# microscopic-image-analysis/geosss

Hardware: AMD Instinct MI355X
Metric: mcmc_chain_steps_per_sec (higher is better)
Workload: dtype f64; 1 GPU; vmfmix_readme: shrinkage slice sampler, 1000000 chains/GPU x 1000 transitions per launch, thin=100; target=vmfmix_readme, d=3, chains_per_gpu=1000000, thin=100, mode=fast, kernel=screened_kernel<3, ScreenVmf<3, 3>>, kept_rows_layout=components, slice_steps=128, library_matches_tree=True, stream=philox-v3 (chain,step)-keyed; S2: tangent = one angle; 32-bit tries

## Files before the change

### geosss_amd/_lib.py

```python
import ctypes as C
import os

_HERE = os.path.dirname(os.path.abspath(__file__))
LIB_PATH = os.environ.get("GSSS_HIP_LIB") or os.path.join(_HERE, "libgsss_hip.so")

VMF_MIXTURE, BINGHAM, CURVE_VMF, CPD, MIXTURE, USER = 1, 2, 3, 4, 5, 6
SHRINK, REJECT, RWMH, HMC, INDEP, MIX = 0, 1, 2, 3, 4, 5
MODE_EXACT, MODE_FAST = 0, 1
VARIANT_FAST_DOUBLE = 100
VARIANT_FAST_VERIFY = 101
CHAIN_MAX_TRIES, CHAIN_NONFINITE, CHAIN_REPLAY_EXHAUSTED, CHAIN_COUNTER_SATURATED = 1, 2, 4, 8
ABI_VERSION = 10
STATS_NO_SECOND_MOMENT = 1
MOMENTS_DIAG = 1


class GsssError(RuntimeError):
    pass


class TargetDesc(C.Structure):
    _fields_ = [("kind", C.c_int32), ("d", C.c_int32), ("k", C.c_int32), ("reserved", C.c_int32),
                ("mu", C.c_void_p), ("logc", C.c_void_p), ("A", C.c_void_p), ("knots", C.c_void_p),
                ("kappa", C.c_double),
                ("source", C.c_void_p), ("source_w", C.c_void_p), ("target", C.c_void_p), ("target_w", C.c_void_p),
                ("n_target", C.c_int32), ("target_dim", C.c_int32), ("k_nn", C.c_int32), ("outlier", C.c_int32),
                ("sigma", C.c_double), ("beta", C.c_double), ("omega", C.c_double), ("log_volume", C.c_double)]


class RunArgs(C.Structure):
    _fields_ = [("state_dev", C.c_void_p), ("samples_dev", C.c_void_p), ("n_reject_dev", C.c_void_p),
                ("n_tries_dev", C.c_void_p), ("err_dev", C.c_void_p), ("replay_dev", C.c_void_p),
                ("replay_stride", C.c_int64), ("n_chains", C.c_int64), ("n_steps", C.c_int64), ("thin", C.c_int64),
                ("seed", C.c_uint64), ("chain_offset", C.c_uint64), ("step_offset", C.c_uint64),
                ("sampler", C.c_int32), ("mode", C.c_int32), ("max_tries", C.c_int32), ("variant", C.c_int32),
                ("rng_state_dev", C.c_void_p), ("samples_chain_rows", C.c_int64), ("placement", C.c_int32),
                ("stats_lags", C.c_int32), ("stats_dev", C.c_void_p), ("stats_dirs_dev", C.c_void_p),
                ("stats_modes", C.c_int32), ("n_leapfrog", C.c_int32), ("stepsize_dev", C.c_void_p),
                ("n_accept_dev", C.c_void_p), ("momenta_dev", C.c_void_p), ("adapt_steps", C.c_int64),
                ("mixing_probability", C.c_double), ("adapt_left_dev", C.c_void_p), ("n_rwmh_dev", C.c_void_p),
                ("momenta_samples_dev", C.c_void_p), ("stepsize_trace_dev", C.c_void_p), ("stats_flags", C.c_int32),
                ("reserved0", C.c_int32)]


SIGNATURES = {
    "gsss_abi_version": (C.c_int, []),
    "gsss_last_error": (C.c_char_p, []),
    "gsss_source_digest": (C.c_char_p, []),
    "gsss_device_count": (C.c_int, []),
    "gsss_target_create": (C.c_int, [C.POINTER(TargetDesc), C.c_int, C.POINTER(C.c_void_p)]),
    "gsss_target_create_mixture": (C.c_int, [C.POINTER(TargetDesc), C.c_int32, C.c_void_p, C.c_int, C.POINTER(C.c_void_p)]),
    "gsss_target_create_batch": (C.c_int, [C.POINTER(TargetDesc), C.c_int32, C.c_int64, C.c_int, C.POINTER(C.c_void_p)]),
    "gsss_exact_layout": (C.c_int, [C.c_int32]),
    "gsss_target_create_user": (C.c_int, [C.c_void_p, C.c_int32, C.c_void_p, C.c_int64, C.c_int, C.POINTER(C.c_void_p)]),
    "gsss_target_destroy": (C.c_int, [C.c_void_p]),
    "gsss_target_dim": (C.c_int, [C.c_void_p]),
    "gsss_logprob": (C.c_int, [C.c_void_p, C.c_void_p, C.c_int64, C.c_void_p, C.c_void_p]),
    "gsss_gradient": (C.c_int, [C.c_void_p, C.c_void_p, C.c_int64, C.c_void_p, C.c_void_p]),
    "gsss_run": (C.c_int, [C.c_void_p, C.POINTER(RunArgs), C.c_void_p]),
    "gsss_stats_rows": (C.c_int64, [C.c_int32, C.c_int32, C.c_int32, C.c_int32]),
    "gsss_moments_rows": (C.c_int64, [C.c_int32, C.c_int32]),
    "gsss_target_moments": (C.c_int, [C.c_void_p, C.c_int64, C.c_int64, C.c_int32, C.c_int64, C.c_int64, C.c_int32, C.c_void_p,
                                      C.c_void_p, C.c_int, C.c_void_p]),
    "gsss_batch_logprob": (C.c_int, [C.c_void_p, C.c_void_p, C.c_int64, C.c_void_p, C.c_void_p]),
    "gsss_batch_gradient": (C.c_int, [C.c_void_p, C.c_void_p, C.c_int64, C.c_void_p, C.c_void_p]),
    "gsss_batch_logprob_draws": (C.c_int, [C.c_void_p, C.c_void_p, C.c_int64, C.c_int64, C.c_int64, C.c_void_p, C.c_void_p]),
    "gsss_scalar_moments": (C.c_int, [C.c_void_p, C.c_int64, C.c_int64, C.c_int64, C.c_void_p, C.c_void_p, C.c_int, C.c_void_p]),
    "gsss_last_launch": (C.c_int, [C.POINTER(C.c_int64), C.POINTER(C.c_int32), C.POINTER(C.c_double)]),
    "gsss_batch_plan": (C.c_int, [C.c_int32, C.c_int32, C.c_int32, C.c_int32, C.c_int64, C.c_int64, C.POINTER(C.c_int32),
                                  C.POINTER(C.c_int32), C.POINTER(C.c_int64), C.POINTER(C.c_double)]),
    "gsss_mode_supported": (C.c_int, [C.c_void_p, C.c_int32]),
    "gsss_variant_name": (C.c_char_p, [C.c_void_p, C.c_int32, C.c_int32]),
    "gsss_kernel_name": (C.c_char_p, [C.c_void_p, C.c_int32, C.c_int32, C.c_int32]),
    "gsss_sample_sphere": (C.c_int, [C.c_uint64, C.c_uint64, C.c_int64, C.c_int32, C.c_void_p, C.c_int, C.c_void_p]),
    "gsss_tangent_s2": (C.c_int, [C.c_void_p, C.c_void_p, C.c_int64, C.c_int32, C.c_void_p, C.c_int, C.c_void_p]),
    "gsss_screen_constants": (C.c_int, [C.POINTER(C.c_double), C.c_int32]),
    "gsss_f32_error_sweep": (C.c_int, [C.c_int32, C.POINTER(C.c_double), C.POINTER(C.c_uint64), C.c_int, C.c_void_p]),
    "gsss_rows_to_components": (C.c_int, [C.c_void_p, C.c_void_p, C.c_int64, C.c_int32, C.c_int, C.c_void_p]),
    "gsss_components_to_rows": (C.c_int, [C.c_void_p, C.c_void_p, C.c_int64, C.c_int32, C.c_int, C.c_void_p]),
    "gsss_samples_to_chains": (C.c_int, [C.c_void_p, C.c_void_p, C.c_int64, C.c_int64, C.c_int32, C.c_int, C.c_void_p]),
    "gsss_malloc": (C.c_int, [C.POINTER(C.c_void_p), C.c_size_t, C.c_int]),
    "gsss_free": (C.c_int, [C.c_void_p, C.c_int]),
    "gsss_memcpy_h2d": (C.c_int, [C.c_void_p, C.c_void_p, C.c_size_t, C.c_int, C.c_void_p]),
    "gsss_memcpy_d2h": (C.c_int, [C.c_void_p, C.c_void_p, C.c_size_t, C.c_int, C.c_void_p]),
    "gsss_malloc_host": (C.c_int, [C.POINTER(C.c_void_p), C.c_size_t, C.c_int]),
    "gsss_free_host": (C.c_int, [C.c_void_p]),
    "gsss_host_register": (C.c_int, [C.c_void_p, C.c_size_t, C.c_int]),
    "gsss_host_unregister": (C.c_int, [C.c_void_p]),
    "gsss_memcpy_d2h_async": (C.c_int, [C.c_void_p, C.c_void_p, C.c_size_t, C.c_int, C.c_void_p]),
    "gsss_memset": (C.c_int, [C.c_void_p, C.c_int, C.c_size_t, C.c_int, C.c_void_p]),
    "gsss_stream_synchronize": (C.c_int, [C.c_int, C.c_void_p]),
}

_lib = None


def load():
    global _lib
    if _lib is not None:
        return _lib
    if not os.path.exists(LIB_PATH):
        raise GsssError(f"{LIB_PATH} is missing: build it with `python -m geosss_amd.build` "
                        "(there is no CPU fallback for the sampler)")
    lib = C.CDLL(LIB_PATH)
    for name, (res, args) in SIGNATURES.items():
        fn = getattr(lib, name)
        fn.restype = res
        fn.argtypes = args
    if lib.gsss_abi_version() != ABI_VERSION:
        raise GsssError(f"libgsss_hip.so has ABI {lib.gsss_abi_version()}, binding expects {ABI_VERSION}")
    _lib = lib
    return lib


def check(code):
    if code != 0:
        msg = load().gsss_last_error().decode("utf-8", "replace")
        if code in (-1, -2):
            raise ValueError(f"gsss: {msg} (code {code})")
        raise GsssError(f"gsss: {msg} (code {code})")


def require_device():
    lib = load()
    n = lib.gsss_device_count()
    if n <= 0:
        raise GsssError("no HIP device visible: the geodesic slice sampler runs on MI355X only "
                        "(no CPU fallback is provided)")
    return n
```

### geosss_amd/csrc/gsss_capi.hip

```cpp
#include <cmath>
#include <cstdarg>
#include <cstdio>
#include <cstring>
#include <mutex>
#include <new>
#include <string>
#include <vector>

#include "gsss_batch.h"
#include "gsss_batch_logprob.h"
#include "gsss_fast.h"
#include "gsss_launch.h"
#include "gsss_mh.h"
#include "gsss_moments.h"
#include "gsss_user_target.h"

namespace gsss {

static thread_local char g_err[512] = "";

static thread_local LaunchInfo g_last_launch = {0, 0, 0.0};
LaunchInfo &last_launch() { return g_last_launch; }

int64_t resident_workgroups(const void *kern, size_t lds_bytes, int *per_cu_out)
{
    struct Entry {
        const void *kern;
        size_t lds;
        int dev, per_cu, cus;
    };
    static std::mutex mu;
    static std::vector<Entry> cache;
    int dev = 0;
    if (hipGetDevice(&dev) != hipSuccess) {
        (void)hipGetLastError();
        return 0;
    }
    const char *env = getenv("GSSS_RESIDENT_PER_CU");
    const int forced = env ? atoi(env) : 0;
    int per_cu = 0, cus = 0;
    {
        std::lock_guard<std::mutex> lock(mu);
        for (const Entry &e : cache)
            if (e.kern == kern && e.lds == lds_bytes && e.dev == dev) {
                per_cu = e.per_cu;
                cus = e.cus;
                break;
            }
    }
    if (per_cu < 1) {
        if (hipOccupancyMaxActiveBlocksPerMultiprocessor(&per_cu, kern, kBlock, lds_bytes) != hipSuccess || per_cu < 1 ||
            hipDeviceGetAttribute(&cus, hipDeviceAttributeMultiprocessorCount, dev) != hipSuccess || cus < 1) {
            (void)hipGetLastError();
            return 0;
        }
        std::lock_guard<std::mutex> lock(mu);
        cache.push_back(Entry{kern, lds_bytes, dev, per_cu, cus});
    }
    if (forced > 0) per_cu = forced;
    if (per_cu_out) *per_cu_out = per_cu;
    return (int64_t)per_cu * cus;
}

void slice_fallback_note(const char *why)
{
    if (getenv("GSSS_DEBUG_OCCUPANCY")) fprintf(stderr, "gsss: %s\n", why);
}

void set_error(const char *fmt, ...)
{
    va_list ap;
    va_start(ap, fmt);
    vsnprintf(g_err, sizeof(g_err), fmt, ap);
    va_end(ap);
}

static const VecInfo kVecs[] = {
#define GSSS_VEC_ROW(ID, V, NAME) {ID, V::L, V::N, V::DPAD, V::kExactDim, NAME},
    GSSS_VEC_LIST(GSSS_VEC_ROW)
#undef GSSS_VEC_ROW
};

const VecInfo *vec_table(int *count)
{
    *count = (int)(sizeof(kVecs) / sizeof(kVecs[0]));
    return kVecs;
}

int select_vec(int d, int variant)
{
    int n;
    const VecInfo *v = vec_table(&n);
    if (variant != 0) {
        for (int i = 0; i < n; ++i)
            if (v[i].id == variant) {
                if (v[i].exact_dim ? v[i].dpad == d : d <= v[i].dpad) return variant;
                set_error("kernel variant %s does not cover d=%d", v[i].name, d);
                return GSSS_E_UNSUPPORTED;
            }
        set_error("unknown kernel variant %d", variant);
        return GSSS_E_INVALID;
    }
    for (int i = 0; i < n; ++i)
        if (v[i].exact_dim && v[i].dpad == d) return v[i].id;
    for (int i = 0; i < n; ++i)
        if (!v[i].exact_dim && d <= v[i].dpad) return v[i].id;
    set_error("no kernel variant covers d=%d (max %d)", d, v[n - 1].dpad);
    return GSSS_E_UNSUPPORTED;
}

static int select_vec_for(const gsss::TargetBlock &tb, int variant)
{
    const int vec = select_vec(tb.d, variant);
    if (vec < 0 || variant != 0) return vec;
    int n;
    const VecInfo *v = vec_table(&n);
    size_t dpad = 0;
    for (int i = 0; i < n; ++i)
        if (v[i].id == vec) dpad = (size_t)v[i].dpad;
    if (dpad >= 256) return vec;
    size_t rows = 0;
    if (tb.kind == GSSS_MIXTURE) {
        int L = 1;
        for (int i = 0; i < n; ++i)
            if (v[i].id == vec) L = v[i].L;
        const MixInfo mi = mix_info(tb);
        const size_t need = (size_t)mi.n * 8 + (L > 1 ? (dpad + 1) * (size_t)(kBlock / L) : 0) + kMixDrawsReserve +
                            (size_t)mi.rows * dpad + (size_t)mi.extra;
        if (need * sizeof(double) <= kMaxLdsBytes) return vec;
        for (int i = 0; i < n; ++i)
            if (!v[i].exact_dim && v[i].dpad >= 256 && tb.d <= v[i].dpad) return v[i].id;
        return vec;
    }
    switch (tb.kind) {
    case GSSS_VMF_MIXTURE: rows = (size_t)tb.k * dpad + (size_t)tb.k; break;
    case GSSS_BINGHAM: rows = (size_t)(tb.d + 1) * dpad; break;
    case GSSS_CURVE_VMF: rows = (size_t)tb.k * dpad + 4 * (size_t)(tb.k - 1); break;
    default: return vec;
    }
    if (rows * sizeof(double) <= gsss::kRowsLdsBytes) return vec;
    for (int i = 0; i < n; ++i)
        if (!v[i].exact_dim && v[i].dpad >= 256 && tb.d <= v[i].dpad) return v[i].id;
    return vec;
}
// ... 981 lines not shown
        const int served = fast_select(fast_ask(t, rb.screen, rb.spread != 0, numpy, replay, rb.stats != nullptr), pick);
        if (numpy && (served != GSSS_OK || !pick.lane)) {
            set_error("in fast mode the numpy stream is served by the lane-per-chain kernels only (gsss_variant_name: "
                      "\"fast-lane\"); use GSSS_MODE_EXACT");
            return GSSS_E_UNSUPPORTED;
        }
        if (a->n_steps > 0x7FFFFFFFll || a->thin > 0x7FFFFFFFll || a->n_chains > 0x7FFFFFFFll - 1024 ||
            a->replay_stride > 0x7FFFFFFFll) {
            set_error("fast mode takes at most 2^31-1 steps / chains per call");
            return GSSS_E_INVALID;
        }
        if (served != GSSS_OK) return fast_refused(t);
        return fast_launch(pick, t->tb, rb, t->batch, replay, st);
    }
    if (mh) {
        if (a->rng_state_dev && (a->sampler == GSSS_RWMH || a->sampler == GSSS_MIX) && t->tb.d < 3) {
            set_error("numpy's gamma(1) is an exponential ziggurat, not restated: RWMH on numpy's stream needs d >= 3");
            return GSSS_E_UNSUPPORTED;
        }
        MhBlock mb;
        mb.stepsize = a->stepsize_dev;
        mb.n_accept = a->n_accept_dev;
        mb.momenta = a->sampler == GSSS_HMC ? a->momenta_dev : nullptr;
        mb.adapt_steps = a->adapt_steps;
        mb.n_leapfrog = a->n_leapfrog;
        mb.kind = a->sampler;
        mb.mix_alpha = a->mixing_probability;
        mb.adapt_left = a->adapt_left_dev;
        mb.n_rwmh = a->n_rwmh_dev;
        mb.momenta_samples = a->sampler == GSSS_HMC ? a->momenta_samples_dev : nullptr;
        mb.stepsize_trace = a->sampler == GSSS_HMC ? nullptr : a->stepsize_trace_dev;
        if (t->tb.kind == GSSS_CPD) return launch_cpd_mh(t->cpd_variant, draws, a->sampler, t->tb, rb, mb, st);
        if (t->tb.kind == GSSS_USER) {
            if (a->sampler == GSSS_HMC && !t->user->has_gradient) {
                set_error("spherical HMC needs the target's gradient: this user target defines no gsss_user_gradient");
                return GSSS_E_UNSUPPORTED;
            }
            return t->user->mh(draws, a->sampler, t->tb, rb, mb, st);
        }
        switch (t->tb.kind) {
        case GSSS_VMF_MIXTURE: return launch_mh<VmfMixture>(vec, draws, a->sampler, t->tb, rb, mb, st);
        case GSSS_BINGHAM: return launch_mh<Bingham>(vec, draws, a->sampler, t->tb, rb, mb, st);
        case GSSS_CURVE_VMF: return launch_mh<CurveVmf>(vec, draws, a->sampler, t->tb, rb, mb, st);
        case GSSS_MIXTURE: return launch_mh<Mixture>(vec, draws, a->sampler, t->tb, rb, mb, st);
        }
        set_error("corrupt target");
        return GSSS_E_INVALID;
    }
    if (t->tb.kind == GSSS_CPD) {
        if (a->stats_dev) {
            set_error("running statistics are not built for registration targets");
            return GSSS_E_UNSUPPORTED;
        }
        return launch_cpd_run(t->cpd_variant, draws, t->tb, rb, st);
    }
    switch (t->tb.kind) {
    case GSSS_VMF_MIXTURE: return launch_run<VmfMixture>(vec, draws, t->tb, rb, st);
    case GSSS_BINGHAM: return launch_run<Bingham>(vec, draws, t->tb, rb, st);
    case GSSS_CURVE_VMF: return launch_run<CurveVmf>(vec, draws, t->tb, rb, st);
    case GSSS_MIXTURE: return launch_run<Mixture>(vec, draws, t->tb, rb, st);
    case GSSS_USER: return t->user->run(draws, t->tb, rb, st);
    }
    set_error("corrupt target");
    return GSSS_E_INVALID;
}

int gsss_batch_plan(int32_t kind, int32_t d, int32_t k, int32_t has_b, int64_t n_targets, int64_t m, int32_t *chains_per_workgroup,
                    int32_t *targets_per_workgroup, int64_t *grid, double *lane_use)
{
    (void)has_b;
    BatchPlan bp;
    if (batch_plan(kind, d, k, n_targets, m, bp) != GSSS_OK) {
        set_error("no fast-mode batch kernel for kind %d, d=%d, k=%d with %lld targets of %lld chains (vMF mixtures: d = 3 .. 10 with "
                  "K <= 16, d = 11 .. 16 with K <= 10; Bingham: d = 3 .. 16)", kind, d, k, (long long)n_targets, (long long)m);
        return GSSS_E_UNSUPPORTED;
    }
    if (chains_per_workgroup) *chains_per_workgroup = bp.per_block;
    if (targets_per_workgroup) *targets_per_workgroup = bp.targets;
    if (grid) *grid = bp.grid;
    if (lane_use) *lane_use = bp.lane_use;
    return GSSS_OK;
}

int gsss_last_launch(int64_t *grid_out, int32_t *slice_steps_out, double *sliced_fraction_out)
{
    if (grid_out) *grid_out = last_launch().grid;
    if (slice_steps_out) *slice_steps_out = last_launch().slice_steps;
    if (sliced_fraction_out) *sliced_fraction_out = last_launch().sliced_fraction;
    return GSSS_OK;
}

int64_t gsss_stats_rows(int32_t d, int32_t n_modes, int32_t n_lags, int32_t flags)
{
    if (d < 2 || n_modes < 0 || n_lags < 0 || (flags & ~GSSS_STATS_NO_SECOND_MOMENT)) return GSSS_E_INVALID;
    const int64_t second = (flags & GSSS_STATS_NO_SECOND_MOMENT) ? 0 : (int64_t)d * (d + 1) / 2;
    return 1 + 2 * (int64_t)d + second + 2 + n_modes + 2 + 3 * (int64_t)n_lags;
}

int64_t gsss_moments_rows(int32_t d, int32_t flags)
{
    if (d < 2 || (flags & ~GSSS_MOMENTS_DIAG)) return GSSS_E_INVALID;
    const bool diag = (flags & GSSS_MOMENTS_DIAG) != 0;
    if (!diag && d > kMomentsMaxFullDim) return GSSS_E_UNSUPPORTED;
    return 1 + moments_sums(d, diag);
}

int gsss_target_moments(const double *samples_dev, int64_t n_rows, int64_t n_chains, int32_t d, int64_t samples_chain_rows,
                        int64_t chains_per_target, int32_t flags, double *acc_dev, double *chain_sum_dev, int device, void *stream)
{
    if (d < 2 || (flags & ~GSSS_MOMENTS_DIAG)) {
        set_error("gsss_target_moments: need d >= 2 and known flags (d = %d, flags = %d)", d, flags);
        return GSSS_E_INVALID;
    }
    if (chains_per_target < 1 || n_chains < 0 || n_chains % chains_per_target != 0) {
        set_error("gsss_target_moments: n_chains (%lld) must be a multiple of chains_per_target (%lld) >= 1", (long long)n_chains,
                  (long long)chains_per_target);
        return GSSS_E_INVALID;
    }
    if (n_rows < 0 || samples_chain_rows < 0 || (samples_chain_rows > 0 && samples_chain_rows < n_rows)) {
        set_error("gsss_target_moments: need n_rows >= 0 and samples_chain_rows 0 or >= n_rows (%lld rows, %lld per chain)",
                  (long long)n_rows, (long long)samples_chain_rows);
        return GSSS_E_INVALID;
    }
    if (!samples_dev || !acc_dev) {
        set_error("gsss_target_moments: %s is null", samples_dev ? "acc_dev" : "samples_dev");
        return GSSS_E_INVALID;
    }
    const bool diag = (flags & GSSS_MOMENTS_DIAG) != 0;
    if (!diag && d > kMomentsMaxFullDim) {
        set_error("gsss_target_moments: the full second-moment triangle is kept for d <= %d (d = %d): pass GSSS_MOMENTS_DIAG",
                  kMomentsMaxFullDim, d);
        return GSSS_E_UNSUPPORTED;
    }
    if (n_rows == 0 || n_chains == 0) return GSSS_OK;
    DeviceGuard guard(device);
    if (!guard.ok) return GSSS_E_HIP;
    return launch_target_moments(samples_dev, n_rows, n_chains, d, samples_chain_rows, chains_per_target, diag, acc_dev, chain_sum_dev,
                                 static_cast<hipStream_t>(stream));
}

int gsss_scalar_moments(const double *values_dev, int64_t n_rows, int64_t n_chains, int64_t chains_per_target, double *acc_dev,
                        double *chain_sum_dev, int device, void *stream)
{
    if (chains_per_target < 1 || n_chains < 0 || n_chains % chains_per_target != 0) {
        set_error("gsss_scalar_moments: n_chains (%lld) must be a multiple of chains_per_target (%lld) >= 1", (long long)n_chains,
                  (long long)chains_per_target);
        return GSSS_E_INVALID;
    }
    if (n_rows < 0) {
        set_error("gsss_scalar_moments: need n_rows >= 0 (%lld)", (long long)n_rows);
        return GSSS_E_INVALID;
    }
    if (n_rows == 0 || n_chains == 0) return GSSS_OK;
    if (!values_dev || !acc_dev) {
        set_error("gsss_scalar_moments: %s is null", values_dev ? "acc_dev" : "values_dev");
        return GSSS_E_INVALID;
    }
    DeviceGuard guard(device);
    if (!guard.ok) return GSSS_E_HIP;
    return launch_target_moments(values_dev, n_rows, n_chains, 1, 0, chains_per_target, true, acc_dev, chain_sum_dev,
                                 static_cast<hipStream_t>(stream));
}

int gsss_mode_supported(const gsss_target *t, int32_t mode)
{
    if (!t) return 0;
// ... 194 lines not shown
```

### geosss_amd/csrc/gsss_device.h

```cpp
#pragma once
#include <hip/hip_runtime.h>
#include <stdint.h>
#include <stdlib.h>

#include "../../include/gsss.h"
#include "gsss_math.h"

namespace gsss {

constexpr int kBlock = 256;
constexpr double kTwoPi = 6.283185307179586;

struct TargetBlock {
    const double *blob;
    int32_t kind, d, k, dpad;
    double kappa;
    double scale;
};

struct RunBlock {
    double *state;
    double *samples;
    int64_t *n_reject;
    int64_t *n_tries;
    int32_t *err;
    const double *replay;
    uint64_t *rng_state;
    int64_t replay_stride;
    int64_t n_chains, n_steps, thin;
    uint64_t seed, chain_offset, step_offset;
    int32_t sampler, max_tries;
    int64_t keep_rows;
    int32_t spread;
    int32_t one_per_lane;
    int32_t stage_rows;
    int32_t screen;
    double *stats;
    const double *stats_dirs;
    int32_t stats_lags, stats_modes;
    int32_t stats_flags;
    int32_t stats_onchip;
    uint32_t *sched;
    int32_t slice_steps;
    int32_t sched_first;
};

struct BatchBlock {
    int64_t stride;
    int32_t m;
    int32_t chunks;
};
struct BatchShared {
    int64_t stride;
    int32_t m;
    int32_t per_block;
};
template <class... BB>
inline constexpr bool kIsBatchShared = false;
template <>
inline constexpr bool kIsBatchShared<BatchShared> = true;
template <class T>
__device__ __forceinline__ const T &first_of(const T &x)
{
    return x;
}

struct SliceSched {
    __device__ static __forceinline__ uint32_t chunks(const RunBlock &a, int per_block) { return (uint32_t)((a.n_chains + per_block - 1) / per_block); }
    __device__ static __forceinline__ uint32_t *progress(const RunBlock &a) { return a.sched + 2; }
    __device__ static __forceinline__ int32_t *dead(const RunBlock &a, int per_block)
    {
        return reinterpret_cast<int32_t *>(a.sched + 2 + chunks(a, per_block));
    }
    __device__ static __forceinline__ bool take(const RunBlock &a, int per_block, uint32_t *word, uint32_t &chunk, int32_t &s_begin,
                                                int32_t &len, bool &timed_out)
    {
        if (threadIdx.x == 0) *word = __hip_atomic_fetch_add(a.sched, 1u, __ATOMIC_RELAXED, __HIP_MEMORY_SCOPE_AGENT);
        __syncthreads();
        const uint32_t t = (uint32_t)__builtin_amdgcn_readfirstlane((int)*word);
        const uint32_t n_chunks = chunks(a, per_block) - (uint32_t)a.sched_first;
        const int32_t ss = a.slice_steps, n_steps = (int32_t)a.n_steps;
        const int32_t first_len = ss - (int32_t)(a.step_offset % (uint64_t)ss);
        const int32_t rest = n_steps - first_len;
        const uint32_t n_items = n_chunks * (uint32_t)(1 + (rest > 0 ? (rest + ss - 1) / ss : 0));
        if (t >= n_items) return false;
        const uint32_t slice = t / n_chunks;
        chunk = (uint32_t)a.sched_first + (t - slice * n_chunks);
        if (threadIdx.x == 0) {
            word[1] = chunk;
            word[2] = slice;
        }
        s_begin = slice == 0 ? 0 : first_len + (int32_t)(slice - 1) * ss;
        int32_t s_end = first_len + (int32_t)slice * ss;
        s_end = s_end < n_steps ? s_end : n_steps;
        len = s_end - s_begin;
        timed_out = false;
        if (slice > 0) {
            __syncthreads();
            if (threadIdx.x == 0) {
                uint32_t ok = 1;
                uint64_t spins = 0;
                const uint64_t limit = (uint64_t)(slice + 1u < 8u ? slice + 1u : 8u) << 22;
                while (__hip_atomic_load(progress(a) + chunk, __ATOMIC_RELAXED, __HIP_MEMORY_SCOPE_AGENT) < slice) {
                    __builtin_amdgcn_s_sleep(32);
                    if (++spins > limit) {
                        ok = 0;
                        break;
                    }
                }
                __builtin_amdgcn_fence(__ATOMIC_ACQUIRE, "agent");
                asm volatile("s_waitcnt vmcnt(0)" ::: "memory");
                *word = ok;
            }
            __syncthreads();
            timed_out = __builtin_amdgcn_readfirstlane((int)*word) == 0;
        }
        return true;
    }
    template <bool kWrittenThrough = false>
    __device__ static __forceinline__ void publish(const RunBlock &a, const uint32_t *word)
    {
        asm volatile("s_waitcnt vmcnt(0)" ::: "memory");
        __syncthreads();
        if (threadIdx.x == 0) {
            if (!kWrittenThrough) {
                __builtin_amdgcn_fence(__ATOMIC_RELEASE, "agent");
                asm volatile("s_waitcnt vmcnt(0)" ::: "memory");
            }
            __hip_atomic_store(progress(a) + word[1], word[2] + 1u, __ATOMIC_RELAXED, __HIP_MEMORY_SCOPE_AGENT);
        }
    }
    template <class T>
    __device__ static __forceinline__ void hand_over(T *p, T v)
    {
        __hip_atomic_store(p, v, __ATOMIC_RELAXED, __HIP_MEMORY_SCOPE_AGENT);
    }
};

constexpr size_t slice_sched_bytes(int64_t n_chunks, int64_t n_chains) { return 4 * (size_t)(2 + n_chunks + n_chains); }

void set_error(const char *fmt, ...);
constexpr size_t kDefaultLdsBytes = 48 * 1024;
constexpr size_t kMaxLdsBytes = 160 * 1024;
constexpr int64_t ceil_div(int64_t a, int64_t b) { return (a + b - 1) / b; }

template <class Kern>
int allow_lds(const char *family, Kern kern, size_t lds)
{
    if (lds <= kDefaultLdsBytes) return GSSS_OK;
    const hipError_t e = hipFuncSetAttribute(reinterpret_cast<const void *>(kern), hipFuncAttributeMaxDynamicSharedMemorySize, (int)lds);
    if (e == hipSuccess) return GSSS_OK;
    set_error("%s kernel: raising its dynamic LDS to %zu B failed: %s", family, lds, hipGetErrorString(e));
    return GSSS_E_HIP;
}

template <class Kern, class... Args>
int launch_kernel(const char *family, Kern kern, int64_t grid, size_t lds, hipStream_t st, void *ws, const Args &...args)
{
    hipLaunchKernelGGL(kern, dim3((unsigned)grid), dim3(kBlock), lds, st, args...);
    const hipError_t e = hipGetLastError();
    if (ws) (void)hipFreeAsync(ws, st);
    if (e == hipSuccess) return GSSS_OK;
    set_error("%s kernel launch failed: %s", family, hipGetErrorString(e));
    return GSSS_E_HIP;
}

struct SlicePlan {
    uint32_t *ws = nullptr;
    int64_t grid = 0;
    int32_t slice_steps = 0;
};
constexpr int kMaxSlices = 64;
inline int slice_length(int64_t n_steps)
{
    const char *env = getenv("GSSS_SLICE_STEPS");
    const int env_val = env ? atoi(env) : 128;
    if (env_val <= 0) return 0;
    int64_t steps = ((int64_t)env_val + 63) / 64 * 64;
    const int64_t floor_steps = ((n_steps + kMaxSlices - 1) / kMaxSlices + 63) / 64 * 64;
    if (steps < floor_steps) steps = floor_steps;
    return steps < 0x40000000ll ? (int)steps : 0;
}
int64_t resident_workgroups(const void *kern, size_t lds_bytes, int *per_cu_out = nullptr);
void slice_fallback_note(const char *why);
struct LaunchInfo {
    int64_t grid;
    int32_t slice_steps;
    double sliced_fraction;
};
LaunchInfo &last_launch();
template <class Kern>
inline SlicePlan plan_slices(Kern kern, size_t lds_bytes, const RunBlock &rb, int64_t n_chunks, bool allowed, hipStream_t st)
{
    SlicePlan p;
    p.grid = n_chunks;
    last_launch() = LaunchInfo{n_chunks, 0, 0.0};
    if (!allowed) return p;
    const int env_steps = slice_length(rb.n_steps);
    if (env_steps <= 0 || rb.n_steps < 2 * (int64_t)env_steps) return p;
    const int64_t resident = resident_workgroups(reinterpret_cast<const void *>(kern), lds_bytes);
    if (resident < 1) return p;
    const int64_t n_slices = 2 + rb.n_steps / env_steps;
    if (n_chunks <= resident || n_chunks * n_slices >= 0x7FFFFFFFll || rb.n_chains >= 0x7FFFFFFFll) return p;
    const size_t bytes = slice_sched_bytes(n_chunks, rb.n_chains);
    void *ws = nullptr;
    if (hipMallocAsync(&ws, bytes, st) != hipSuccess || ws == nullptr) {
        (void)hipGetLastError();
        slice_fallback_note("hipMallocAsync of the slice workspace failed: launching unsliced");
        return p;
    }
    if (hipMemsetAsync(ws, 0, bytes, st) != hipSuccess) {
        (void)hipGetLastError();
        (void)hipFreeAsync(ws, st);
        return p;
    }
    const int64_t first_len = env_steps - (int64_t)(rb.step_offset % (uint64_t)env_steps), rest = rb.n_steps - first_len;
    p.ws = static_cast<uint32_t *>(ws);
    p.grid = n_chunks * (1 + (rest > 0 ? (rest + env_steps - 1) / env_steps : 0));
    p.slice_steps = env_steps;
    last_launch() = LaunchInfo{p.grid, p.slice_steps, 1.0};
    return p;
}

template <class Kern>
inline SlicePlan plan_partial_round(Kern kern, size_t lds_bytes, const RunBlock &rb, int64_t n_chunks, bool allowed, hipStream_t st,
                                    int32_t &first_out)
{
    SlicePlan p;
    p.grid = n_chunks;
    first_out = 0;
    last_launch() = LaunchInfo{n_chunks, 0, 0.0};
    if (!allowed) return p;
    const int env_steps = slice_length(rb.n_steps);
    if (env_steps <= 0 || rb.n_steps < 2 * (int64_t)env_steps) return p;
    const int64_t resident = resident_workgroups(reinterpret_cast<const void *>(kern), lds_bytes);
    if (resident < 1) return p;
    const int64_t rem = n_chunks % resident, first = n_chunks - rem;
    if (n_chunks <= resident || rem == 0 || 4 * rem > 3 * resident || rb.n_chains >= 0x7FFFFFFFll) return p;
    const int64_t first_len = env_steps - (int64_t)(rb.step_offset % (uint64_t)env_steps), rest = rb.n_steps - first_len;
    const int64_t n_slices = 1 + (rest > 0 ? (rest + env_steps - 1) / env_steps : 0);
    if (rem * n_slices >= 0x7FFFFFFFll) return p;
    const size_t bytes = slice_sched_bytes(n_chunks, rb.n_chains);
    void *ws = nullptr;
    if (hipMallocAsync(&ws, bytes, st) != hipSuccess || ws == nullptr) {
        (void)hipGetLastError();
        slice_fallback_note("hipMallocAsync of the slice workspace failed: launching unsliced");
        return p;
    }
    if (hipMemsetAsync(ws, 0, bytes, st) != hipSuccess) {
        (void)hipGetLastError();
        (void)hipFreeAsync(ws, st);
        return p;
    }
    p.ws = static_cast<uint32_t *>(ws);
    p.grid = first + rem * n_slices;
    p.slice_steps = env_steps;
    first_out = (int32_t)first;
    last_launch() = LaunchInfo{p.grid, p.slice_steps, (double)rem / (double)n_chunks};
    return p;
}

__device__ __forceinline__ size_t sample_index(const RunBlock &a, int64_t row, int j, int d, int64_t c)
{
    return a.keep_rows > 0 ? ((size_t)c * a.keep_rows + row) * d + j : ((size_t)row * d + j) * a.n_chains + c;
}

template <int D>
__device__ __forceinline__ void stats_update(const RunBlock &a, int64_t c, const double (&x)[D])
{
    const size_t n = (size_t)a.n_chains;
    double *s = a.stats + c;
    const int K = a.stats_modes, L = a.stats_lags;
    const bool second = !(a.stats_flags & GSSS_STATS_NO_SECOND_MOMENT);
    const int T = second ? D * (D + 1) / 2 : 0;
    const int r_prev = 1, r_sum = 1 + D, r_xx = 1 + 2 * D, r_dist = r_xx + T, r_hop = r_dist + 1, r_mode = r_hop + 1;
    const int r_p = r_mode + K, r_lag = r_p + 2, r_ring = r_lag + L, r_head = r_ring + L;
    const double *w = a.stats_dirs, *h = a.stats_dirs + D, *modes = a.stats_dirs + 2 * D;
    const int64_t cnt = (int64_t)s[0];
    double p = 0.0, xh = 0.0;
#pragma unroll
    for (int j = 0; j < D; ++j) {
        p = fma(x[j], w[j], p);
        xh = fma(x[j], h[j], xh);
    }
    if (cnt > 0) {
        double dot = 0.0, ph = 0.0;
#pragma unroll
        for (int j = 0; j < D; ++j) {
            const double pj = s[(size_t)(r_prev + j) * n];
            dot = fma(pj, x[j], dot);
            ph = fma(pj, h[j], ph);
        }
        s[(size_t)r_dist * n] += acos(fmin(fmax(dot, -1.0), 1.0));
        const int sa = (xh > 0.0) - (xh < 0.0), sb = (ph > 0.0) - (ph < 0.0);
        if (sa != sb) s[(size_t)r_hop * n] += 1.0;
    }
    int t = 0;
#pragma unroll
    for (int i = 0; i < D; ++i) {
        s[(size_t)(r_prev + i) * n] = x[i];
        s[(size_t)(r_sum + i) * n] += x[i];
        if (second) {
#pragma unroll
            for (int j = i; j < D; ++j) s[(size_t)(r_xx + t++) * n] += x[i] * x[j];
        }
    }
    if (K > 0) {
        int best = 0;
        double bv = -INFINITY;
        for (int k = 0; k < K; ++k) {
            double v = 0.0;
#pragma unroll
            for (int j = 0; j < D; ++j) v = fma(x[j], modes[k * D + j], v);
            if (v > bv) {
                bv = v;
// ... 1434 lines not shown
```

### geosss_amd/csrc/gsss_screen.h

```cpp
#pragma once
#include <type_traits>

#include "gsss_fast.h"
#include "gsss_screen_consts.h"

namespace gsss {

enum : int32_t { kFinalAccept = 3, kFinalDecide = 4, kFinalInHi = 2 };
__device__ __forceinline__ bool is_final(int32_t st) { return st >= kFinalAccept; }
__device__ __forceinline__ bool is_decide(int32_t st) { return st == kFinalDecide || st == kFinalDecide + kFinalInHi; }

__device__ __forceinline__ void sincos_rev32(double theta, float &s, float &c)
{
    const float t = (float)(theta * 0.15915494309189535);
    s = __builtin_amdgcn_sinf(t);
    c = __builtin_amdgcn_cosf(t);
}

__device__ __forceinline__ float log2_32(double v)
{
    int e;
    const double m = frexp(v, &e);
    return (float)e + __builtin_amdgcn_logf((float)m);
}
// ... 565 lines not shown
        if (__hip_atomic_fetch_add(&gsss_svc_ticket, 1u, __ATOMIC_ACQ_REL, __HIP_MEMORY_SCOPE_AGENT) == waves - 1) {
            unsigned long long s[8];
            for (int i = 0; i < 8; ++i) s[i] = __hip_atomic_exchange(&gsss_svc_count[i], 0ull, __ATOMIC_RELAXED, __HIP_MEMORY_SCOPE_AGENT);
            __hip_atomic_store(&gsss_svc_ticket, 0u, __ATOMIC_RELAXED, __HIP_MEMORY_SCOPE_AGENT);
            printf("gsss-svc phases %llu decide_phases %llu decides %llu decide_accepts %llu finalised %llu setups %llu "
                   "try_iters %llu all_idle_accept_phases %llu\n", s[0], s[1], s[2], s[3], s[4], s[5], s[6], s[7]);
        }
    }
}
#endif

__device__ __forceinline__ void lds_trade(float &a, int32_t &b, unsigned long long *slot)
{
    const unsigned long long mine = (unsigned long long)__float_as_uint(a) | ((unsigned long long)(uint32_t)b << 32);
    const unsigned long long o = __hip_atomic_exchange(slot, mine, __ATOMIC_RELAXED, __HIP_MEMORY_SCOPE_WORKGROUP);
    a = __uint_as_float((uint32_t)o);
    b = (int32_t)(uint32_t)(o >> 32);
}

__device__ __forceinline__ bool divides(int32_t n, int32_t d, double rcp, int32_t &quot)
{
    int32_t q = (int32_t)((double)n * rcp);
    int32_t r = n - q * d;
    if (r < 0) {
        --q;
        r += d;
    }
    if (r >= d) {
        ++q;
        r -= d;
    }
    quot = q;
    return r == 0;
}

__device__ __forceinline__ void lds_trade(float &a, float &b, unsigned long long *slot)
{
    const unsigned long long mine = (unsigned long long)__float_as_uint(a) | ((unsigned long long)__float_as_uint(b) << 32);
    const unsigned long long o = __hip_atomic_exchange(slot, mine, __ATOMIC_RELAXED, __HIP_MEMORY_SCOPE_WORKGROUP);
    a = __uint_as_float((uint32_t)o);
    b = __uint_as_float((uint32_t)(o >> 32));
}

template <class TP, bool SHARED>
__host__ __device__ constexpr int screen_min_waves()
{
    if constexpr (SHARED)
        return TP::kSharedMinWaves;
    else
        return TP::kMinWaves;
}

template <int D, class TP, bool REPLAY, bool STATS = false, bool STAGE = false, bool NUMPY = false, bool BATCH = false, class... BB>
__global__ void __launch_bounds__(kBlock, (STATS || (REPLAY && !NUMPY)) ? 1 : (NUMPY ? TP::kNumpyWaves : screen_min_waves<TP, kIsBatchShared<BB...>>()))
    screened_kernel(TargetBlock tb, RunBlock a, BB... batch)
{
    static_assert(!NUMPY || (REPLAY && !STAGE), "numpy's stream is a sequential source: it is read where the replay buffer is");
    static_assert(sizeof...(BB) == (BATCH ? 1 : 0) && !(BATCH && (REPLAY || STATS || STAGE || NUMPY)),
                  "the batch build takes one BatchBlock (or BatchShared): library stream, no running statistics");
    using V = LaneVec<D>;
    using Chain = ScreenChain<D, TP>;
    extern __shared__ __attribute__((aligned(16))) double lds[];
    TP tp;
    constexpr bool kShared = kIsBatchShared<BB...>;
    [[maybe_unused]] int32_t shared_id = 0;
    if constexpr (kShared) {
        shared_id = stage_shared(tp, lds, tb, first_of(batch...), (int32_t)a.n_chains);
    } else {
        if constexpr (BATCH) tb.blob += (int64_t)(blockIdx.x / (uint32_t)first_of(batch...).chunks) * first_of(batch...).stride;
        tp.stage(lds, tb);
    }
    const fm::Tables tab = stage_tables(kShared ? lds : lds + TP::lds_doubles());
    unsigned long long *park = reinterpret_cast<unsigned long long *>(lds + TP::lds_doubles() + kTabLds) + threadIdx.x;
    NumpyDraws<V> nd;
    if constexpr (NUMPY) nd.stage(lds + TP::lds_doubles() + kTabLds);
    constexpr int kStageP = (!STAGE || !TP::kHoldRows || D % 4 == 0) ? 1 : ((D % 2 == 0) ? 2 : 4);
    double *stage = reinterpret_cast<double *>(park);
    int32_t n_staged = 0;
    __syncthreads();

    const int32_t n = (int32_t)a.n_chains;
    constexpr int kChunk = (screen_parks<D, TP>() && !NUMPY && !STAGE && !BATCH) ? 2 * kBlock : kBlock;
    __shared__ uint32_t sched_word[4];
    const bool sliced = a.sched != nullptr && (int32_t)blockIdx.x >= a.sched_first;
    uint32_t chunk = blockIdx.x;
    int32_t s_begin = 0, n_steps = (int32_t)a.n_steps;
    bool timed_out = false;
    if (sliced) {
        int32_t len;
        if (!SliceSched::take(a, a.one_per_lane ? kBlock : kChunk, sched_word, chunk, s_begin, len, timed_out)) return;
        n_steps = s_begin + len;
    }
    const bool shrink = a.sampler == GSSS_SHRINK;
    const int32_t thin = (int32_t)a.thin;
    const double rcp_thin = 1.0 / (double)thin;
    const int32_t max_tries = a.max_tries < (1 << 25) ? a.max_tries : (1 << 25) - 1;
    constexpr uint32_t kTryBase = 1u + (uint32_t)((D + 3) / 4);
    constexpr bool kPark = screen_parks<D, TP>() && !NUMPY && !STAGE && !BATCH;
    constexpr int kPerBlock = kPark ? 2 * kBlock : kBlock;
    int32_t id0 = (int32_t)chunk * (a.one_per_lane ? kBlock : kPerBlock) + (int32_t)threadIdx.x;
    if constexpr (kShared) {
        id0 = shared_id;
    } else if constexpr (BATCH) {
        const BatchBlock &bb = first_of(batch...);
        const uint32_t t = blockIdx.x / (uint32_t)bb.chunks, l = blockIdx.x - t * (uint32_t)bb.chunks;
        const int64_t id = (int64_t)t * bb.m + (int64_t)l * kBlock + (int64_t)threadIdx.x;
        id0 = (id < ((int64_t)t + 1) * bb.m && id < (int64_t)n) ? (int32_t)id : n;
    }
    const int32_t id1 = a.one_per_lane ? n : id0 + kBlock;

    Chain cur;
    int32_t slot = 0;
    int32_t parked_status = kDone;
    StatsLane<D> sl;
    const bool stats_onchip = STATS && a.stats_onchip > 0;

    auto chain_id = [&]() { return slot ? id1 : id0; };
    auto philox = [&]() {
        PhiloxDraws<V, true> dr;
        dr.tab = tab;
        dr.init(a, chain_id(), D);
        dr.begin_step(a.step_offset + (uint64_t)cur.steps_done);
        return dr;
    };
    auto replay_take = [&]() -> double {
        if constexpr (NUMPY) return nd.next_double();
        if (cur.cursor >= (int32_t)a.replay_stride) {
            cur.err |= GSSS_CHAIN_REPLAY_EXHAUSTED;
            return 0.5;
        }
        return a.replay[(size_t)chain_id() * a.replay_stride + cur.cursor++];
    };
    auto count_tries = [&]() {
        const uint32_t sum = cur.n_try + (uint32_t)cur.t;
        if (sum < cur.n_try) cur.err |= GSSS_CHAIN_COUNTER_SATURATED;
        cur.n_try = sum < cur.n_try ? 0xFFFFFFFFu : sum;
    };
    auto needs_service = [](int32_t st) { return st == kPending || is_final(st); };

    auto init = [&]() {
        const int32_t c = chain_id();
        const bool valid = c < n;
        const int32_t cc = valid ? c : 0;
#pragma unroll
        for (int j = 0; j < D; ++j) cur.x[j] = a.state[(size_t)j * n + cc];
#pragma unroll
        for (int j = 0; j < D; ++j) cur.u[j] = 0.0;
#pragma unroll
        for (int i = 0; i < Chain::kQ; ++i) cur.q[i] = 0.0f;
        cur.lo = cur.hi = cur.thr = 0.0;
        cur.n_try = 0u;
        cur.steps_done = s_begin;
        cur.row = s_begin / thin;
        cur.err = 0;
        cur.cursor = 0;
        cur.t = 0;
        cur.status = (valid && n_steps > s_begin) ? kPending : kDone;
        if constexpr (NUMPY) nd.init(a, cc, D);
        if constexpr (STATS) {
            if (stats_onchip && valid) sl.load(a, cc, reinterpret_cast<double *>(park));
        }
        if (sliced && valid) {
            if (SliceSched::dead(a, a.one_per_lane ? kBlock : kChunk)[cc] != 0) cur.status = kDone;
            if (timed_out && cur.status != kDone) {
                cur.err |= GSSS_CHAIN_MAX_TRIES | GSSS_CHAIN_COUNTER_SATURATED;
                cur.status = kDone;
            }
        }
    };

    auto setup = [&]() {
        double u_thr, u_th0;
        uint32_t w_phi = 0u;
// ... 487 lines not shown
```

### include/gsss.h

```cpp
#ifndef GSSS_H
#define GSSS_H

#include <stddef.h>
#include <stdint.h>

#ifdef __cplusplus
extern "C" {
#endif

#define GSSS_ABI_VERSION 10

#define GSSS_VMF_MIXTURE 1
#define GSSS_BINGHAM 2
#define GSSS_CURVE_VMF 3
#define GSSS_CPD 4
#define GSSS_MIXTURE 5
#define GSSS_USER 6

#define GSSS_SHRINK 0
#define GSSS_REJECT 1
#define GSSS_RWMH 2
#define GSSS_HMC 3
#define GSSS_INDEP 4
#define GSSS_MIX 5
// ... 27 lines not shown
    const double *mu;
    const double *logc;
    const double *A;
    const double *knots;
    double kappa;
    const double *source;
    const double *source_w;
    const double *target;
    const double *target_w;
    int32_t n_target;
    int32_t target_dim;
    int32_t k_nn;
    int32_t outlier;
    double sigma;
    double beta;
    double omega;
    double log_volume;
} gsss_target_desc;

typedef struct gsss_run_args {
    double *state_dev;
    double *samples_dev;
    int64_t *n_reject_dev;
    int64_t *n_tries_dev;
    int32_t *err_dev;
    const double *replay_dev;
    int64_t replay_stride;
    int64_t n_chains;
    int64_t n_steps;
    int64_t thin;
    uint64_t seed;
    uint64_t chain_offset;
    uint64_t step_offset;
    int32_t sampler;
    int32_t mode;
    int32_t max_tries;
    int32_t variant;
    uint64_t *rng_state_dev;
    int64_t samples_chain_rows;
    int32_t placement;
    int32_t stats_lags;
    double *stats_dev;
    const double *stats_dirs_dev;
    int32_t stats_modes;
    int32_t n_leapfrog;
    double *stepsize_dev;
    int64_t *n_accept_dev;
    double *momenta_dev;
    int64_t adapt_steps;
    double mixing_probability;
    int64_t *adapt_left_dev;
    int64_t *n_rwmh_dev;
    double *momenta_samples_dev;
    double *stepsize_trace_dev;
    int32_t stats_flags;
    int32_t reserved0;
} gsss_run_args;

int gsss_abi_version(void);
const char *gsss_last_error(void);

const char *gsss_source_digest(void);

int gsss_device_count(void);

int gsss_target_create(const gsss_target_desc *desc, int device, gsss_target **out);
int gsss_target_create_mixture(const gsss_target_desc *components, int32_t n_components, const double *log_weights, int device,
                               gsss_target **out);
int gsss_target_create_batch(const gsss_target_desc *targets, int32_t n_targets, int64_t chains_per_target, int device,
                             gsss_target **out);
int gsss_exact_layout(int32_t d);
int gsss_target_create_user(const void *table, int32_t d, const double *params, int64_t n_params, int device, gsss_target **out);
int gsss_target_destroy(gsss_target *t);
int gsss_target_dim(const gsss_target *t);

int gsss_logprob(const gsss_target *t, const double *x_dev, int64_t n, double *out_dev, void *stream);

int gsss_gradient(const gsss_target *t, const double *x_dev, int64_t n, double *grad_dev, void *stream);

int gsss_run(const gsss_target *t, const gsss_run_args *args, void *stream);

int gsss_last_launch(int64_t *grid_out, int32_t *slice_steps_out, double *sliced_fraction_out);

int gsss_batch_plan(int32_t kind, int32_t d, int32_t k, int32_t has_b, int64_t n_targets, int64_t m,
                    int32_t *chains_per_workgroup, int32_t *targets_per_workgroup, int64_t *grid, double *lane_use);

int64_t gsss_stats_rows(int32_t d, int32_t n_modes, int32_t n_lags, int32_t flags);

#define GSSS_MOMENTS_DIAG 1
int64_t gsss_moments_rows(int32_t d, int32_t flags);
int gsss_target_moments(const double *samples_dev, int64_t n_rows, int64_t n_chains, int32_t d, int64_t samples_chain_rows,
                        int64_t chains_per_target, int32_t flags, double *acc_dev, double *chain_sum_dev, int device, void *stream);

int gsss_batch_logprob(const gsss_target *t, const double *x_dev, int64_t n_per_target, double *out_dev, void *stream);
int gsss_batch_gradient(const gsss_target *t, const double *x_dev, int64_t n_per_target, double *grad_dev, void *stream);
int gsss_batch_logprob_draws(const gsss_target *t, const double *samples_dev, int64_t n_rows, int64_t n_chains, int64_t target0,
                             double *out_dev, void *stream);
int gsss_scalar_moments(const double *values_dev, int64_t n_rows, int64_t n_chains, int64_t chains_per_target, double *acc_dev,
                        double *chain_sum_dev, int device, void *stream);

int gsss_mode_supported(const gsss_target *t, int32_t mode);

const char *gsss_variant_name(const gsss_target *t, int32_t mode, int32_t variant);
const char *gsss_kernel_name(const gsss_target *t, int32_t mode, int32_t variant, int32_t placement);

int gsss_sample_sphere(uint64_t seed, uint64_t chain_offset, int64_t n, int32_t d, double *state_dev, int device,
                       void *stream);

int gsss_tangent_s2(const double *x_dev, const uint32_t *w_dev, int64_t n, int32_t table_driven, double *out_dev, int device,
                    void *stream);

int gsss_screen_constants(double *out, int32_t n);
int gsss_f32_error_sweep(int32_t which, double *out_host, uint64_t *n_swept_out, int device, void *stream);

int gsss_rows_to_components(const double *in_dev, double *out_dev, int64_t n, int32_t d, int device, void *stream);
int gsss_components_to_rows(const double *in_dev, double *out_dev, int64_t n, int32_t d, int device, void *stream);
int gsss_samples_to_chains(const double *in_dev, double *out_dev, int64_t n, int64_t n_keep, int32_t d, int device,
                           void *stream);

int gsss_malloc(void **out_dev, size_t bytes, int device);
int gsss_free(void *p_dev, int device);
int gsss_memcpy_h2d(void *dst_dev, const void *src_host, size_t bytes, int device, void *stream);
int gsss_memcpy_d2h(void *dst_host, const void *src_dev, size_t bytes, int device, void *stream);
int gsss_memset(void *dst_dev, int value, size_t bytes, int device, void *stream);
int gsss_malloc_host(void **out_host, size_t bytes, int device);
int gsss_free_host(void *p_host);
int gsss_host_register(void *p_host, size_t bytes, int device);
int gsss_host_unregister(void *p_host);
int gsss_memcpy_d2h_async(void *dst_host, const void *src_dev, size_t bytes, int device, void *stream);
int gsss_stream_synchronize(int device, void *stream);

#ifdef __cplusplus
}
#endif
#endif
```

Before: 49.45 billion chain-steps/s.

## Balance tail wave with precomputed piece table splitting chunks across resident workgroups

Adds a host-planned table that cuts the total chunk×step work into equal spans per resident workgroup, splitting chunks at step boundaries into head and tail pieces. Workgroups fetch pieces by atomic ticket, and tail pieces spin-wait until the head piece of the same chunk has published its progress. This targets the idle last wave when the chunk count is not a multiple of the number of resident workgroups. The cost is a cached pinned table, an async workspace allocation and copy, and spin-wait dependencies between pieces.

```diff
diff --git a/geosss_amd/_lib.py b/geosss_amd/_lib.py
--- a/geosss_amd/_lib.py
+++ b/geosss_amd/_lib.py
@@ -69,6 +69,7 @@
     "gsss_last_launch": (C.c_int, [C.POINTER(C.c_int64), C.POINTER(C.c_int32), C.POINTER(C.c_double)]),
     "gsss_batch_plan": (C.c_int, [C.c_int32, C.c_int32, C.c_int32, C.c_int32, C.c_int64, C.c_int64, C.POINTER(C.c_int32),
                                   C.POINTER(C.c_int32), C.POINTER(C.c_int64), C.POINTER(C.c_double)]),
+    "gsss_piece_plan": (C.c_int64, [C.c_int64, C.c_int64, C.c_int64, C.POINTER(C.c_int32), C.c_int64]),
     "gsss_mode_supported": (C.c_int, [C.c_void_p, C.c_int32]),
     "gsss_variant_name": (C.c_char_p, [C.c_void_p, C.c_int32, C.c_int32]),
     "gsss_kernel_name": (C.c_char_p, [C.c_void_p, C.c_int32, C.c_int32, C.c_int32]),
diff --git a/geosss_amd/csrc/gsss_capi.hip b/geosss_amd/csrc/gsss_capi.hip
--- a/geosss_amd/csrc/gsss_capi.hip
+++ b/geosss_amd/csrc/gsss_capi.hip
@@ -60,6 +60,38 @@
     if (forced > 0) per_cu = forced;
     if (per_cu_out) *per_cu_out = per_cu;
     return (int64_t)per_cu * cus;
+}
+
+const Piece *piece_table_staged(int64_t n_chunks, int64_t resident, int64_t n_steps, int64_t *count_out, int64_t *split_out)
+{
+    struct Entry {
+        int64_t n_chunks, resident, n_steps, count, split;
+        Piece *table;
+    };
+    constexpr size_t kMaxTables = 256;
+    static std::mutex mu;
+    static std::vector<Entry> cache;
+    std::lock_guard<std::mutex> lock(mu);
+    for (const Entry &e : cache)
+        if (e.n_chunks == n_chunks && e.resident == resident && e.n_steps == n_steps) {
+            *count_out = e.count;
+            *split_out = e.split;
+            return e.table;
+        }
+    if (cache.size() >= kMaxTables) return nullptr;
+    int64_t split = 0;
+    const std::vector<Piece> table = piece_plan(n_chunks, resident, n_steps, &split);
+    if (table.empty()) return nullptr;
+    void *host = nullptr;
+    if (hipHostMalloc(&host, table.size() * sizeof(Piece), hipHostMallocPortable) != hipSuccess || host == nullptr) {
+        (void)hipGetLastError();
+        return nullptr;
+    }
+    memcpy(host, table.data(), table.size() * sizeof(Piece));
+    cache.push_back(Entry{n_chunks, resident, n_steps, (int64_t)table.size(), split, static_cast<Piece *>(host)});
+    *count_out = (int64_t)table.size();
+    *split_out = split;
+    return cache.back().table;
 }
 
 void slice_fallback_note(const char *why)
@@ -1207,6 +1239,24 @@
     return GSSS_OK;
 }
 
+int64_t gsss_piece_plan(int64_t n_chunks, int64_t resident, int64_t n_steps, int32_t *table_out, int64_t capacity)
+{
+    if (n_chunks < 1 || resident < 1 || n_steps < 1 || capacity < 0) {
+        set_error("gsss_piece_plan: need n_chunks, resident, n_steps >= 1 and capacity >= 0 (%lld, %lld, %lld, %lld)", (long long)n_chunks,
+                  (long long)resident, (long long)n_steps, (long long)capacity);
+        return GSSS_E_INVALID;
+    }
+    const std::vector<Piece> table = piece_plan(n_chunks, resident, n_steps);
+    if (table_out != nullptr) {
+        if ((int64_t)table.size() > capacity) {
+            set_error("gsss_piece_plan: the table has %lld pieces, the buffer holds %lld", (long long)table.size(), (long long)capacity);
+            return GSSS_E_INVALID;
+        }
+        if (!table.empty()) memcpy(table_out, table.data(), table.size() * sizeof(Piece));
+    }
+    return (int64_t)table.size();
+}
+
 int gsss_last_launch(int64_t *grid_out, int32_t *slice_steps_out, double *sliced_fraction_out)
 {
     if (grid_out) *grid_out = last_launch().grid;
diff --git a/geosss_amd/csrc/gsss_device.h b/geosss_amd/csrc/gsss_device.h
--- a/geosss_amd/csrc/gsss_device.h
+++ b/geosss_amd/csrc/gsss_device.h
@@ -2,6 +2,9 @@
 #include <hip/hip_runtime.h>
 #include <stdint.h>
 #include <stdlib.h>
+
+#include <algorithm>
+#include <vector>
 
 #include "../../include/gsss.h"
 #include "gsss_math.h"
@@ -65,6 +68,7 @@
     return x;
 }
 
+enum PieceKind : int32_t { kPieceWhole = 0, kPieceHead = 1, kPieceTail = 2 };
 struct SliceSched {
     __device__ static __forceinline__ uint32_t chunks(const RunBlock &a, int per_block) { return (uint32_t)((a.n_chains + per_block - 1) / per_block); }
     __device__ static __forceinline__ uint32_t *progress(const RunBlock &a) { return a.sched + 2; }
@@ -117,6 +121,50 @@
         }
         return true;
     }
+    __device__ static __forceinline__ const uint32_t *pieces(const RunBlock &a, int per_block)
+    {
+        const size_t words = 2 + (size_t)chunks(a, per_block) + (size_t)a.n_chains;
+        return a.sched + ((words + 3) & ~(size_t)3);
+    }
+    __device__ static __forceinline__ bool take_piece(const RunBlock &a, int per_block, uint32_t *word, uint32_t &chunk, int32_t &s_begin,
+                                                      int32_t &len, int32_t &kind, bool &timed_out)
+    {
+        if (threadIdx.x == 0) *word = __hip_atomic_fetch_add(a.sched, 1u, __ATOMIC_RELAXED, __HIP_MEMORY_SCOPE_AGENT);
+        __syncthreads();
+        const uint32_t t = (uint32_t)__builtin_amdgcn_readfirstlane((int)*word);
+        if (t >= gridDim.x) return false;
+        const uint32_t *e = pieces(a, per_block) + 4 * (size_t)t;
+        chunk = e[0];
+        s_begin = (int32_t)e[1];
+        len = (int32_t)e[2];
+        kind = (int32_t)e[3];
+        if (threadIdx.x == 0) {
+            word[1] = chunk;
+            word[2] = 0u;
+        }
+        timed_out = false;
+        if (kind == kPieceTail) {
+            __syncthreads();
+            if (threadIdx.x == 0) {
+                uint32_t ok = 1;
+                uint64_t spins = 0;
+                const uint64_t limit = (uint64_t)2u << 22;
+                while (__hip_atomic_load(progress(a) + chunk, __ATOMIC_RELAXED, __HIP_MEMORY_SCOPE_AGENT) < 1u) {
+                    __builtin_amdgcn_s_sleep(32);
+                    if (++spins > limit) {
+                        ok = 0;
+                        break;
+                    }
+                }
+                __builtin_amdgcn_fence(__ATOMIC_ACQUIRE, "agent");
+                asm volatile("s_waitcnt vmcnt(0)" ::: "memory");
+                *word = ok;
+            }
+            __syncthreads();
+            timed_out = __builtin_amdgcn_readfirstlane((int)*word) == 0;
+        }
+        return true;
+    }
     template <bool kWrittenThrough = false>
     __device__ static __forceinline__ void publish(const RunBlock &a, const uint32_t *word)
     {
@@ -222,6 +270,73 @@
     return p;
 }
 
+constexpr int32_t kPieceMin = 32;
+constexpr int64_t kPieceMinSteps = 256;
+struct Piece {
+    int32_t chunk, s_begin, len, kind;
+};
+static_assert(sizeof(Piece) == 16, "a table entry is four words");
+inline bool piece_plan_applies(int64_t n_chunks, int64_t resident, int64_t n_steps)
+{
+    return resident >= 1 && n_chunks > resident && n_chunks % resident != 0 && n_steps >= kPieceMinSteps && n_steps < 0x40000000ll &&
+           n_chunks < 0x40000000ll;
+}
+inline std::vector<Piece> piece_plan(int64_t n_chunks, int64_t resident, int64_t n_steps, int64_t *split_out = nullptr)
+{
+    std::vector<Piece> table;
+    if (split_out) *split_out = 0;
+    if (!piece_plan_applies(n_chunks, resident, n_steps)) return table;
+    const int64_t C = n_chunks, R = resident, N = n_steps, W = C * N;
+    struct Planned {
+        int64_t start, slot;
+        Piece piece;
+    };
+    std::vector<Planned> planned;
+    planned.reserve((size_t)(C + R));
+    int64_t lo = 0, split = 0;
+    for (int64_t j = 0; j < R; ++j) {
+        int64_t hi = W;
+        if (j + 1 < R) {
+            hi = (j + 1) * (W / R) + (j + 1) * (W % R) / R;
+            const int64_t x = hi % N;
+            if (x < kPieceMin)
+                hi -= x;
+            else if (N - x < kPieceMin)
+                hi -= kPieceMin - (N - x);
+            const int64_t pc = lo / N, px = lo % N;
+            const int64_t floor_pos = px ? (pc + 1) * N : lo;
+            if (hi < floor_pos) hi = floor_pos;
+            if (px && hi / N == pc + 1 && hi % N != 0 && hi % N < px) hi = (pc + 1) * N + px;
+        }
+        for (int64_t p = lo; p < hi;) {
+            const int64_t c = p / N, x = p % N;
+            const int64_t end = (c + 1) * N < hi ? (c + 1) * N : hi;
+            Piece e;
+            e.chunk = (int32_t)c;
+            if (x) {
+                e.s_begin = 0, e.len = (int32_t)(N - x), e.kind = kPieceHead;
+            } else if (end - p < N) {
+                e.s_begin = (int32_t)(N - (end - p)), e.len = (int32_t)(end - p), e.kind = kPieceTail;
+                ++split;
+            } else {
+                e.s_begin = 0, e.len = (int32_t)N, e.kind = kPieceWhole;
+            }
+            planned.push_back(Planned{p - lo, j, e});
+            p = end;
+        }
+        lo = hi;
+    }
+    std::stable_sort(planned.begin(), planned.end(), [](const Planned &a, const Planned &b) { return a.start != b.start ? a.start < b.start : a.slot < b.slot; });
+    table.reserve(planned.size());
+    for (const Planned &p : planned) table.push_back(p.piece);
+    if (split_out) *split_out = split;
+    return table;
+}
+
+const Piece *piece_table_staged(int64_t n_chunks, int64_t resident, int64_t n_steps, int64_t *count_out, int64_t *split_out);
+constexpr bool kPiecePlanDefault = true;
+constexpr size_t piece_table_offset(int64_t n_chunks, int64_t n_chains) { return (slice_sched_bytes(n_chunks, n_chains) + 15) / 16 * 16; }
+
 template <class Kern>
 inline SlicePlan plan_partial_round(Kern kern, size_t lds_bytes, const RunBlock &rb, int64_t n_chunks, bool allowed, hipStream_t st,
                                     int32_t &first_out)
@@ -231,6 +346,35 @@
     first_out = 0;
     last_launch() = LaunchInfo{n_chunks, 0, 0.0};
     if (!allowed) return p;
+    const char *env_pieces = getenv("GSSS_PIECE_PLAN");
+    if (getenv("GSSS_SLICE_STEPS") == nullptr && (env_pieces ? env_pieces[0] != '0' : kPiecePlanDefault)) {
+        const int64_t resident = resident_workgroups(reinterpret_cast<const void *>(kern), lds_bytes);
+        if (!piece_plan_applies(n_chunks, resident, rb.n_steps) || rb.n_chains >= 0x7FFFFFFFll) return p;
+        int64_t count = 0, split = 0;
+        const Piece *table = piece_table_staged(n_chunks, resident, rb.n_steps, &count, &split);
+        if (table == nullptr || count < 1) {
+            slice_fallback_note("no page-locked memory for the piece table: launching one workgroup per chunk");
+            return p;
+        }
+        const size_t head_bytes = piece_table_offset(n_chunks, rb.n_chains), bytes = head_bytes + (size_t)count * sizeof(Piece);
+        void *ws = nullptr;
+        if (hipMallocAsync(&ws, bytes, st) != hipSuccess || ws == nullptr) {
+            (void)hipGetLastError();
+            slice_fallback_note("hipMallocAsync of the piece workspace failed: launching one workgroup per chunk");
+            return p;
+        }
+        if (hipMemsetAsync(ws, 0, head_bytes, st) != hipSuccess ||
+            hipMemcpyAsync(static_cast<char *>(ws) + head_bytes, table, (size_t)count * sizeof(Piece), hipMemcpyHostToDevice, st) != hipSuccess) {
+            (void)hipGetLastError();
+            (void)hipFreeAsync(ws, st);
+            return p;
+        }
+        p.ws = static_cast<uint32_t *>(ws);
+        p.grid = count;
+        p.slice_steps = 0;
+        last_launch() = LaunchInfo{count, (int32_t)((rb.n_steps + 1) / 2), (double)split / (double)n_chunks};
+        return p;
+    }
     const int env_steps = slice_length(rb.n_steps);
     if (env_steps <= 0 || rb.n_steps < 2 * (int64_t)env_steps) return p;
     const int64_t resident = resident_workgroups(reinterpret_cast<const void *>(kern), lds_bytes);
diff --git a/geosss_amd/csrc/gsss_screen.h b/geosss_amd/csrc/gsss_screen.h
--- a/geosss_amd/csrc/gsss_screen.h
+++ b/geosss_amd/csrc/gsss_screen.h
@@ -671,13 +671,18 @@
     const int32_t n = (int32_t)a.n_chains;
     constexpr int kChunk = (screen_parks<D, TP>() && !NUMPY && !STAGE && !BATCH) ? 2 * kBlock : kBlock;
     __shared__ uint32_t sched_word[4];
-    const bool sliced = a.sched != nullptr && (int32_t)blockIdx.x >= a.sched_first;
+    bool sliced = a.sched != nullptr && (int32_t)blockIdx.x >= a.sched_first;
     uint32_t chunk = blockIdx.x;
     int32_t s_begin = 0, n_steps = (int32_t)a.n_steps;
     bool timed_out = false;
     if (sliced) {
         int32_t len;
-        if (!SliceSched::take(a, a.one_per_lane ? kBlock : kChunk, sched_word, chunk, s_begin, len, timed_out)) return;
+        if (a.slice_steps == 0) {
+            int32_t kind;
+            if (!SliceSched::take_piece(a, a.one_per_lane ? kBlock : kChunk, sched_word, chunk, s_begin, len, kind, timed_out)) return;
+            sliced = kind != kPieceWhole;
+        } else if (!SliceSched::take(a, a.one_per_lane ? kBlock : kChunk, sched_word, chunk, s_begin, len, timed_out))
+            return;
         n_steps = s_begin + len;
     }
     const bool shrink = a.sampler == GSSS_SHRINK;
diff --git a/include/gsss.h b/include/gsss.h
--- a/include/gsss.h
+++ b/include/gsss.h
@@ -133,6 +133,8 @@
 
 int gsss_last_launch(int64_t *grid_out, int32_t *slice_steps_out, double *sliced_fraction_out);
 
+int64_t gsss_piece_plan(int64_t n_chunks, int64_t resident, int64_t n_steps, int32_t *table_out, int64_t capacity);
+
 int gsss_batch_plan(int32_t kind, int32_t d, int32_t k, int32_t has_b, int64_t n_targets, int64_t m,
                     int32_t *chains_per_workgroup, int32_t *targets_per_workgroup, int64_t *grid, double *lane_use);
 
```

After: 51.06 billion chain-steps/s, median of 6. 3.3% higher.
